# TinfoilHat0/Defending-Against-Backdoors-with-Robust-Learning-Rate

Hardware: NVIDIA H100
Metric: fl_rounds_per_sec (higher is better)
Workload: dtype bf16

## Files before the change

### defending-against-backdoors-with-robust-learning-rate_b200/ops/csrc/gemm.h

```cpp
#pragma once
#include <cuda_runtime.h>
#include <cuda_bf16.h>
#include <stdint.h>

#include "dropspec.h"

namespace rlr {

constexpr int kStatSlots = 16;

struct ConvGemmParams {
    int M, N, num_kb;
    int mode;
    int cblocks;
    int TW, TH, TN;
    int Ho, Wo, NB;
    int tiles_w, tiles_h;
    int ntaps;
    int in_stride;
    int out_stride, out_ph, out_pw, OutH, OutW;
    int8_t dh[9], dw[9];
    int dn[9];
    int b_mn;
    int wtap[9];
    int wcols;
    DropSpec drop;
    int tma_store;
    int split_prod;
    long long* dbg;
    const __nv_bfloat16* b_src;
    int b_ld, b_kvalid;
    const uint32_t* wait_flags;
    int wait_lo, wait_hi;
    const uint32_t* wait_epoch;
    void* out;
    int ldc;
    const float* bias;
    float* stats;
    int stat_slots;
    int relu, accumulate;
};

cudaError_t launch_gemm_bf16(const void* A, const void* B, void* out, int M, int N, int K, int lda, int ldb, int ldc,
                             const float* bias, int relu, int accumulate, float* stats, cudaStream_t st, const DropSpec* drop = nullptr);
cudaError_t launch_stem_gemm_bf16(const void* A, const void* W, void* out, int M, int N, int kvalid, int ldw, const float* bias, int relu,
                                  float* stats, const uint32_t* wait_flags, int wait_lo, int wait_hi, const uint32_t* wait_epoch,
                                  cudaStream_t st);
void set_pdl(int on);
cudaError_t launch_gemm_splitk_bf16(const void* A, const void* B, void* out, float* ws, int M, int N, int K, const float* bias, int relu,
                                    int num_sms, cudaStream_t st, const DropSpec* drop = nullptr);
void set_persistent_conv(int on);
void set_conv_occ3(int level);
void set_conv_tma_store(int on);
void set_conv_split_producer(int on);
void set_conv_trace(long long* buf);
long long* conv_trace_buf();
cudaError_t launch_conv_bf16(const void* x, const void* w, void* out, int NB, int planes, int Hin, int Win, int Cin, int Ho, int Wo,
                             int Cout, int ldc, int ntaps, const int* dh, const int* dw, const int* dplane, const float* bias,
                             int relu, int accumulate, float* stats, cudaStream_t st, const int* wtap = nullptr, int w_taps_total = 0,
                             int in_stride = 1, int out_stride = 1, int out_ph = 0, int out_pw = 0);

cudaError_t launch_conv3x3_halo_bf16(const void* x, const void* w, void* out, int NB, int Hin, int Win, int H, int W, int Cout, const float* bias,
                                     int relu, int accumulate, float* stats, int bo_mode, long long* dbg, int num_sms, cudaStream_t st);

cudaError_t launch_conv3x3_halo3_bf16(const void* x, const void* w, void* out, int NB, int H, int W, int Cout, const float* bias, int relu,
                                      int accumulate, int num_sms, cudaStream_t st);

cudaError_t launch_conv_wgrad_bf16(const void* dy, const void* x, float* dW, int NB, int planes, int Hin, int Win, int Cin, int Cin_valid,
                                   int Ho, int Wo, int Cout, int ntaps, const int* dh, const int* dw, const int* dplane, int num_sms,
                                   cudaStream_t st, int in_stride = 1);
cudaError_t launch_conv_wgrad_halo_bf16(const void* dy, const void* x, float* dW, int NB, int H, int W, int Cin_valid, int Cout,
                                        int num_sms, cudaStream_t st);
cudaError_t launch_linear_wgrad_bf16(const void* dy, const void* x, float* dW, int B, int N, int K, int num_sms, cudaStream_t st);

cudaError_t launch_ordered_sum_f32(float* out, const float* part, int nparts, long long n, cudaStream_t st);
cudaError_t launch_ordered_sum_f64(double* out, const double* part, int nparts, long long n, cudaStream_t st);
cudaError_t launch_channel_stats(const __nv_bfloat16* x, long long M, int C, float* stats , int num_sms, cudaStream_t st,
                                 int only_sum = 0, int nslots = 1);
cudaError_t launch_bn_finalize(const float* stats, int slots, float* mean_rstd, float* running_mean, float* running_var, int C,
                               float count, float eps, float momentum, int train, cudaStream_t st);
cudaError_t launch_bn_apply(const __nv_bfloat16* x, const __nv_bfloat16* res, __nv_bfloat16* y, const float* gamma, const float* beta,
                            float* mean_rstd, long long M, int C, int relu, int fin_mode, const float* stats, int slots, float count,
                            float eps, float momentum, float* running_mean, float* running_var, int num_sms, cudaStream_t st);
cudaError_t launch_bn_bwd_reduce(const __nv_bfloat16* dy, const __nv_bfloat16* y, const __nv_bfloat16* x, const float* mean_rstd,
                                 float* dsum , long long M, int C, int relu, int num_sms, cudaStream_t st,
                                 const float* gamma = nullptr, const float* beta = nullptr, int nslots = 1);
cudaError_t launch_bn_bwd_apply(const __nv_bfloat16* dy, const __nv_bfloat16* y, const __nv_bfloat16* x, const float* gamma,
                                const float* mean_rstd, const float* dsum, __nv_bfloat16* dx, __nv_bfloat16* dres, float* dgamma,
                                float* dbeta, long long M, int C, int relu, int num_sms, cudaStream_t st, const float* beta = nullptr, int nslots = 1);
cudaError_t launch_gn_fwd(const __nv_bfloat16* x, const __nv_bfloat16* res, __nv_bfloat16* y, const float* gamma, const float* beta,
                          float* mean_rstd, int B, int HW, int C, int G, float eps, int relu, int num_sms, cudaStream_t st);
cudaError_t launch_gn_bwd(const __nv_bfloat16* dy, const __nv_bfloat16* y, const __nv_bfloat16* x, const float* gamma,
                          const float* mean_rstd, __nv_bfloat16* dx, __nv_bfloat16* dres, float* dgamma, float* dbeta, int B, int HW,
                          int C, int G, int relu, int num_sms, cudaStream_t st);
cudaError_t launch_relu_bwd(__nv_bfloat16* dy, const __nv_bfloat16* y, long long n, int num_sms, cudaStream_t st, float scale = 1.0f);
cudaError_t launch_maxpool2_fwd(const __nv_bfloat16* x, __nv_bfloat16* y, uint8_t* idx, int B, int H, int W, int C, cudaStream_t st,
                                float drop_p = 0.f, uint64_t seed = 0, const long long* step = nullptr, uint64_t stream = 0);
cudaError_t launch_maxpool2_bwd(const __nv_bfloat16* dy, const uint8_t* idx, __nv_bfloat16* dx, int B, int H, int W, int C, cudaStream_t st,
                                float drop_p, uint64_t seed, const long long* step, uint64_t stream, const __nv_bfloat16* zmask);
cudaError_t launch_avgpool_fwd(const __nv_bfloat16* x, __nv_bfloat16* y, int B, int HW, int C, cudaStream_t st);
cudaError_t launch_avgpool_bwd(const __nv_bfloat16* dy, __nv_bfloat16* dx, int B, int HW, int C, cudaStream_t st);
cudaError_t launch_dropout_fwd(const __nv_bfloat16* x, __nv_bfloat16* y, uint8_t* mask, long long n, float p, uint64_t seed,
                               const long long* step, uint64_t stream, cudaStream_t st);
cudaError_t launch_dropout_bwd(const __nv_bfloat16* dy, const uint8_t* mask, __nv_bfloat16* dx, long long n, float p, cudaStream_t st);
cudaError_t launch_space_to_depth(const __nv_bfloat16* x, __nv_bfloat16* y, int NB, int H, int W, int C, int num_sms, cudaStream_t st);
cudaError_t launch_im2col_small(const __nv_bfloat16* x, __nv_bfloat16* A, int NB, int H, int W, int C, int Ho, int Wo, int k, int pad,
                                int num_sms, cudaStream_t st);
cudaError_t launch_depth_to_space(const __nv_bfloat16* x4, __nv_bfloat16* y, int NB, int H, int W, int C, int accumulate, int plane_mask,
                                  int num_sms, cudaStream_t st);
cudaError_t launch_filter_gather_transpose(const __nv_bfloat16* w, __nv_bfloat16* wt, int Cout, int T, int Cin, int nsub, const int* taps,
                                           cudaStream_t st);
cudaError_t launch_filter_transpose(const __nv_bfloat16* w, __nv_bfloat16* wt, int Cout, int ntaps, int Cin, cudaStream_t st);
cudaError_t launch_linear_small_fwd(const __nv_bfloat16* x, const __nv_bfloat16* w, const float* bias, __nv_bfloat16* y, int B, int K,
                                    int N, int relu, cudaStream_t st);
cudaError_t launch_linear_small_fwd2(const __nv_bfloat16* x, const __nv_bfloat16* w, const float* bias, __nv_bfloat16* y, int B, int K,
                                     int N, int relu, cudaStream_t st);
cudaError_t launch_linear_small_bwd2(const __nv_bfloat16* x, const __nv_bfloat16* dy, const __nv_bfloat16* w, __nv_bfloat16* dx,
                                     float* dw, float* db, int B, int K, int N, int accumulate_dx, cudaStream_t st);
cudaError_t launch_linear_small_bwd(const __nv_bfloat16* x, const __nv_bfloat16* dy, const __nv_bfloat16* w, __nv_bfloat16* dx,
                                    float* dw, float* db, int B, int K, int N, int accumulate_dx, cudaStream_t st);

}
```

### defending-against-backdoors-with-robust-learning-rate_b200/ops/csrc/gemm_binding.cpp

```cpp
#include <torch/extension.h>
#include <ATen/cuda/CUDAContext.h>
#include <c10/cuda/CUDAGuard.h>
#include <c10/cuda/CUDAStream.h>
#include <c10/cuda/CUDACachingAllocator.h>

#include <vector>

#include "gemm.h"

namespace rlr {
void* scratch_alloc(size_t bytes, cudaStream_t st) {
    return c10::cuda::CUDACachingAllocator::raw_alloc_with_stream(bytes < 256 ? 256 : bytes, st);
}
void scratch_free(void* p) { c10::cuda::CUDACachingAllocator::raw_delete(p); }
}

namespace {
inline cudaStream_t cur_stream() { return c10::cuda::getCurrentCUDAStream().stream(); }
inline int num_sms() { return at::cuda::getCurrentDeviceProperties()->multiProcessorCount; }
inline void check(cudaError_t e, const char* what) { TORCH_CHECK(e == cudaSuccess, what, ": ", cudaGetErrorString(e)); }
template <typename T>
inline T* opt(const c10::optional<at::Tensor>& t) { return t.has_value() && t->defined() ? reinterpret_cast<T*>(t->data_ptr()) : nullptr; }
inline const __nv_bfloat16* bf(const at::Tensor& t) {
    TORCH_CHECK(t.is_cuda() && t.scalar_type() == at::kBFloat16 && t.is_contiguous(), "expected contiguous CUDA bf16 tensor");
// ... 252 lines not shown
    check(rlr::launch_maxpool2_fwd(bf(x), bfm(y), (uint8_t*)idx.data_ptr(), x.size(0), x.size(1), x.size(2), x.size(3), cur_stream(),
                                   (float)drop_p, d.seed, d.step, d.stream), "maxpool2_fwd");
}
void maxpool2_bwd(at::Tensor dy, at::Tensor idx, at::Tensor dx, double drop_p, int64_t drop_seed, c10::optional<at::Tensor> drop_step, int64_t drop_stream,
                  c10::optional<at::Tensor> relu_out) {
    c10::cuda::CUDAGuard g(dx.device());
    const rlr::DropSpec d = drop_spec(drop_p, drop_seed, drop_step, drop_stream);
    const bool zm = relu_out.has_value() && relu_out->defined();
    TORCH_CHECK(!zm || (relu_out->scalar_type() == at::kBFloat16 && relu_out->is_contiguous() && relu_out->numel() == dy.numel()), "relu_out must match dy");
    TORCH_CHECK(dy.is_contiguous() && dx.is_contiguous() && idx.is_contiguous() && dy.size(1) == dx.size(1) / 2 && dy.size(2) == dx.size(2) / 2);
    check(rlr::launch_maxpool2_bwd(bf(dy), (const uint8_t*)idx.data_ptr(), bfm(dx), dx.size(0), dx.size(1), dx.size(2), dx.size(3), cur_stream(),
                                   (float)drop_p, d.seed, d.step, d.stream, zm ? bf(*relu_out) : nullptr), "maxpool2_bwd");
}
void avgpool_fwd(at::Tensor x, at::Tensor y) {
    c10::cuda::CUDAGuard g(x.device());
    check(rlr::launch_avgpool_fwd(bf(x), bfm(y), x.size(0), x.size(1) * x.size(2), x.size(3), cur_stream()), "avgpool_fwd");
}
void avgpool_bwd(at::Tensor dy, at::Tensor dx) {
    c10::cuda::CUDAGuard g(dx.device());
    check(rlr::launch_avgpool_bwd(bf(dy), bfm(dx), dx.size(0), dx.size(1) * dx.size(2), dx.size(3), cur_stream()), "avgpool_bwd");
}
void dropout_fwd(at::Tensor x, at::Tensor y, at::Tensor mask, double p, int64_t seed, at::Tensor step, int64_t stream) {
    c10::cuda::CUDAGuard g(x.device());
    check(rlr::launch_dropout_fwd(bf(x), bfm(y), (uint8_t*)mask.data_ptr(), x.numel(), (float)p, (uint64_t)seed,
                                  (const long long*)step.data_ptr(), (uint64_t)stream, cur_stream()), "dropout_fwd");
}
void dropout_bwd(at::Tensor dy, at::Tensor mask, at::Tensor dx, double p) {
    c10::cuda::CUDAGuard g(dx.device());
    check(rlr::launch_dropout_bwd(bf(dy), (const uint8_t*)mask.data_ptr(), bfm(dx), dx.numel(), (float)p, cur_stream()), "dropout_bwd");
}
void space_to_depth(at::Tensor x, at::Tensor y) {
    c10::cuda::CUDAGuard g(x.device());
    check(rlr::launch_space_to_depth(bf(x), bfm(y), x.size(0), x.size(1), x.size(2), x.size(3), num_sms(), cur_stream()), "space_to_depth");
}
void im2col_small(at::Tensor x, at::Tensor A, int64_t k, int64_t pad) {
    c10::cuda::CUDAGuard g(x.device());
    const int NB = x.size(0), H = x.size(1), W = x.size(2), C = x.size(3);
    const int Ho = H + 2 * pad - k + 1, Wo = W + 2 * pad - k + 1;
    TORCH_CHECK(x.dim() == 4 && x.is_contiguous() && A.is_contiguous() && A.numel() == (int64_t)NB * Ho * Wo * 64, "im2col_small: A must be [NB*Ho*Wo, 64]");
    check(rlr::launch_im2col_small(bf(x), bfm(A), NB, H, W, C, Ho, Wo, (int)k, (int)pad, num_sms(), cur_stream()), "im2col_small");
}
void depth_to_space(at::Tensor x4, at::Tensor y, bool accumulate, int64_t plane_mask) {
    c10::cuda::CUDAGuard g(y.device());
    check(rlr::launch_depth_to_space(bf(x4), bfm(y), y.size(0), y.size(1), y.size(2), y.size(3), accumulate, (int)plane_mask, num_sms(),
                                     cur_stream()), "depth_to_space");
}
void filter_gather_transpose(at::Tensor w, at::Tensor wt, int64_t Cout, int64_t T, int64_t Cin, std::vector<int64_t> taps) {
    c10::cuda::CUDAGuard g(w.device());
    int t[9];
    TORCH_CHECK(taps.size() >= 1 && taps.size() <= 9);
    for (size_t i = 0; i < taps.size(); ++i) t[i] = (int)taps[i];
    check(rlr::launch_filter_gather_transpose(bf(w), bfm(wt), Cout, T, Cin, (int)taps.size(), t, cur_stream()), "filter_gather_transpose");
}
void filter_transpose(at::Tensor w, at::Tensor wt, int64_t Cout, int64_t ntaps, int64_t Cin) {
    c10::cuda::CUDAGuard g(w.device());
    check(rlr::launch_filter_transpose(bf(w), bfm(wt), Cout, ntaps, Cin, cur_stream()), "filter_transpose");
}
void linear_small_fwd(at::Tensor x, at::Tensor w, c10::optional<at::Tensor> bias, at::Tensor y, bool relu) {
    c10::cuda::CUDAGuard g(x.device());
    check(rlr::launch_linear_small_fwd(bf(x), bf(w), opt<const float>(bias), bfm(y), x.size(0), x.size(1), w.size(0), relu, cur_stream()), "linear_small_fwd");
}
void linear_small_bwd(at::Tensor x, at::Tensor dy, at::Tensor w, c10::optional<at::Tensor> dx, at::Tensor dw, c10::optional<at::Tensor> db,
                      bool accumulate_dx) {
    c10::cuda::CUDAGuard g(x.device());
    check(rlr::launch_linear_small_bwd(bf(x), bf(dy), bf(w), const_cast<__nv_bfloat16*>(bfo(dx)), (float*)dw.data_ptr(), opt<float>(db),
                                       x.size(0), x.size(1), w.size(0), accumulate_dx, cur_stream()), "linear_small_bwd");
}
void linear_small_fwd2(at::Tensor x, at::Tensor w, c10::optional<at::Tensor> bias, at::Tensor y, bool relu) {
    c10::cuda::CUDAGuard g(x.device());
    check(rlr::launch_linear_small_fwd2(bf(x), bf(w), opt<const float>(bias), bfm(y), x.size(0), x.size(1), w.size(0), relu, cur_stream()), "linear_small_fwd2");
}
void linear_small_bwd2(at::Tensor x, at::Tensor dy, at::Tensor w, c10::optional<at::Tensor> dx, at::Tensor dw, c10::optional<at::Tensor> db,
                       bool accumulate_dx) {
    c10::cuda::CUDAGuard g(x.device());
    check(rlr::launch_linear_small_bwd2(bf(x), bf(dy), bf(w), const_cast<__nv_bfloat16*>(bfo(dx)), (float*)dw.data_ptr(), opt<float>(db),
                                        x.size(0), x.size(1), w.size(0), accumulate_dx, cur_stream()), "linear_small_bwd2");
}
}

void register_gemm_bindings(py::module_& m) {
    m.attr("STAT_SLOTS") = rlr::kStatSlots;
    m.def("set_persistent_conv", [](bool on) { rlr::set_persistent_conv(on ? 1 : 0); });
    m.def("set_pdl", [](bool on) { rlr::set_pdl(on ? 1 : 0); });
    m.def("set_conv_occ3", [](int64_t level) { rlr::set_conv_occ3((int)level); });
    m.def("set_conv_tma_store", [](bool on) { rlr::set_conv_tma_store(on ? 1 : 0); });
    m.def("set_conv_split_producer", [](bool on) { rlr::set_conv_split_producer(on ? 1 : 0); });
    m.def("set_conv_trace", [](c10::optional<at::Tensor> buf) {
        rlr::set_conv_trace(buf.has_value() && buf->defined() ? reinterpret_cast<long long*>(buf->data_ptr<int64_t>()) : nullptr);
    });
    m.def("gemm_bf16", &gemm_bf16, py::arg("A"), py::arg("B"), py::arg("out"), py::arg("bias"), py::arg("relu"), py::arg("accumulate"), py::arg("stats"),
          py::arg("drop_p") = 0.0, py::arg("drop_seed") = 0, py::arg("drop_step") = py::none(), py::arg("drop_stream") = 0);
    m.def("stem_gemm_bf16", &stem_gemm_bf16, py::arg("A"), py::arg("W"), py::arg("out"), py::arg("bias"), py::arg("relu"), py::arg("stats"),
          py::arg("ready_ptr") = 0, py::arg("lo") = 0, py::arg("hi") = 0, py::arg("epoch") = py::none());
    m.def("gemm_splitk_bf16", &gemm_splitk_bf16, py::arg("A"), py::arg("B"), py::arg("out"), py::arg("ws"), py::arg("bias"), py::arg("relu"),
          py::arg("drop_p") = 0.0, py::arg("drop_seed") = 0, py::arg("drop_step") = py::none(), py::arg("drop_stream") = 0);
    m.def("conv_bf16", &conv_bf16);
    m.def("conv_bf16_strided", &conv_bf16_strided);
    m.def("conv_wgrad_bf16_strided", &conv_wgrad_bf16_strided);
    m.def("conv3x3_halo_bf16", &conv3x3_halo_bf16);
    m.def("conv3x3_halo3_bf16", &conv3x3_halo3_bf16);
    m.def("conv_wgrad_bf16", &conv_wgrad_bf16);
    m.def("linear_wgrad_bf16", &linear_wgrad_bf16);
    m.def("conv_wgrad_halo_bf16", &conv_wgrad_halo_bf16);
    m.def("channel_stats", &channel_stats);
    m.def("ordered_sum", &ordered_sum);
    m.def("bias_grad", &bias_grad);
    m.def("bn_finalize", &bn_finalize);
    m.def("bn_apply", &bn_apply);
    m.def("bn_bwd", &bn_bwd);
    m.def("bn_bwd_recompute", &bn_bwd_recompute);
    m.def("gn_fwd", &gn_fwd);
    m.def("gn_bwd", &gn_bwd);
    m.def("relu_bwd", &relu_bwd, py::arg("dy"), py::arg("y"), py::arg("scale") = 1.0);
    m.def("maxpool2_fwd", &maxpool2_fwd, py::arg("x"), py::arg("y"), py::arg("idx"), py::arg("drop_p") = 0.0, py::arg("drop_seed") = 0,
          py::arg("drop_step") = py::none(), py::arg("drop_stream") = 0);
    m.def("maxpool2_bwd", &maxpool2_bwd, py::arg("dy"), py::arg("idx"), py::arg("dx"), py::arg("drop_p") = 0.0, py::arg("drop_seed") = 0,
          py::arg("drop_step") = py::none(), py::arg("drop_stream") = 0, py::arg("relu_out") = py::none());
    m.def("avgpool_fwd", &avgpool_fwd);
    m.def("avgpool_bwd", &avgpool_bwd);
    m.def("dropout_fwd", &dropout_fwd);
    m.def("dropout_bwd", &dropout_bwd);
    m.def("space_to_depth", &space_to_depth);
    m.def("im2col_small", &im2col_small);
    m.def("filter_transpose", &filter_transpose);
    m.def("depth_to_space", &depth_to_space);
    m.def("filter_gather_transpose", &filter_gather_transpose);
    m.def("linear_small_fwd", &linear_small_fwd);
    m.def("linear_small_bwd", &linear_small_bwd);
    m.def("linear_small_fwd2", &linear_small_fwd2);
    m.def("linear_small_bwd2", &linear_small_bwd2);
}
```

### defending-against-backdoors-with-robust-learning-rate_b200/ops/csrc/wgrad.cu

```cuda
#include <cuda.h>
#include <stdlib.h>

#include "common.cuh"
#include "gemm.h"
#include "wgmma.cuh"

namespace rlr {

using namespace wg;

cudaError_t make_tmap_bf16(CUtensorMap* map, const void* base, int rank, const uint64_t* dims, const uint64_t* strides_bytes,
                           const uint32_t* box, const uint32_t* elem_strides = nullptr);

constexpr int WG_BM = 128, WG_BK = 64;
constexpr int WG_STAGES = 3;
constexpr int WG_A_BYTES = 2 * 64 * WG_BK * 2;
constexpr int WG_THREADS = 256 + 32;
template <int BNW>
struct WgCfg {
    static constexpr int kGroups = BNW / 64;
    static constexpr int kBBytes = kGroups * 64 * WG_BK * 2;
    static constexpr int kStageBytes = WG_A_BYTES + 3 * kBBytes;
    static constexpr int kSmem = WG_STAGES * kStageBytes + 2048;
};

struct WgradParams {
    int mode;
    int num_kb;
    int kb_per_cta;
    int a_groups;
    int ntaps_cta;
    int T;
    int TW, TH, TN, tiles_w, tiles_h;
    int8_t dh[9], dw[9];
    int dn[9];
    int in_stride;
    int ci_tiles;
    int Cout, Cin_valid;
    float* dW;
    float* part;
};

struct __align__(8) WgShared {
    uint64_t full[WG_STAGES];
    uint64_t empty[WG_STAGES];
};

template <int NACC, int BNW>
__device__ __forceinline__ void wgrad_flush(const float (&acc)[NACC / 2], float* dW, float* part, int co, int Cout, int T, int tap0, int ci0,
                                            int Cin_valid, int t) {
    if (part) dW = part + (size_t)blockIdx.z * Cout * T * Cin_valid;
#pragma unroll
    for (int h = 0; h < 2; ++h) {
        const int row = co + 8 * h;
        if (row >= Cout) continue;
#pragma unroll
        for (int j = 0; j < NACC / 8; ++j) {
            const int c = frag_col(t, 4 * j), tap = c / BNW, ci = ci0 + c % BNW;
            float* dst = dW + ((size_t)row * T + tap0 + tap) * Cin_valid + ci;
            const float a = acc[4 * j + 2 * h], b = acc[4 * j + 2 * h + 1];
            if (part) {
                if (ci < Cin_valid) dst[0] = a;
                if (ci + 1 < Cin_valid) dst[1] = b;
            } else if ((Cin_valid & 1) == 0) {
                if (ci < Cin_valid) asm volatile("red.global.add.v2.f32 [%0], {%1, %2};" ::"l"(dst), "f"(a), "f"(b) : "memory");
            } else {
                if (ci < Cin_valid) atomicAdd(dst, a);
                if (ci + 1 < Cin_valid) atomicAdd(dst + 1, b);
            }
        }
    }
}

template <int BNW, int kTaps>
__global__ void __launch_bounds__(WG_THREADS, 1)
umma_wgrad_kernel(const __grid_constant__ CUtensorMap tmA, const __grid_constant__ CUtensorMap tmB, const WgradParams p) {
    using Cfg = WgCfg<BNW>;
    constexpr int WG_BN = BNW, WG_B_BYTES = Cfg::kBBytes, WG_STAGE_BYTES = Cfg::kStageBytes;
    constexpr int NACC = kTaps * BNW;
    extern __shared__ uint8_t smem_raw[];
    uint8_t* smem = reinterpret_cast<uint8_t*>((reinterpret_cast<uintptr_t>(smem_raw) + 1023) & ~uintptr_t(1023));
    WgShared* sh = reinterpret_cast<WgShared*>(smem + WG_STAGES * WG_STAGE_BYTES);
    const int warp = threadIdx.x >> 5, lane = threadIdx.x & 31;
    const int co_tile = blockIdx.x / p.ci_tiles, ci_tile = blockIdx.x - co_tile * p.ci_tiles;
    const int tap0 = blockIdx.y * kTaps;
    const int kb_begin = blockIdx.z * p.kb_per_cta;
    const int kb_end = min(p.num_kb, kb_begin + p.kb_per_cta);
    const int nkb = kb_end - kb_begin;

    if (warp == 8 && lane == 0) {
        prefetch_tmap(&tmA); prefetch_tmap(&tmB);
        for (int s = 0; s < WG_STAGES; ++s) { mbar_init(&sh->full[s], 1); mbar_init(&sh->empty[s], 8); }
        fence_barrier_init();
    }
    __syncthreads();
    pdl_wait();
    pdl_trigger();

    if (warp == 8) {
        if (lane == 0) {
            int stage = 0;
            uint32_t phase = 0;
            const uint32_t bytes = p.a_groups * 8192 + kTaps * WG_B_BYTES;
            for (int i = 0; i < nkb; ++i) {
                const int kb = kb_begin + i;
                mbar_wait(&sh->empty[stage], phase ^ 1);
                uint8_t* sa = smem + stage * WG_STAGE_BYTES;
                uint8_t* sb = sa + WG_A_BYTES;
                mbar_expect_tx(&sh->full[stage], bytes);
                if (p.mode == 1) {
                    const int tw_i = kb % p.tiles_w, th_i = (kb / p.tiles_w) % p.tiles_h, tn_i = kb / (p.tiles_w * p.tiles_h);
                    const int w0 = tw_i * p.TW, h0 = th_i * p.TH, n0 = tn_i * p.TN;
                    for (int g = 0; g < p.a_groups; ++g)
                        tma_load_4d(&tmA, &sh->full[stage], sa + g * 8192, co_tile * WG_BM + g * 64, w0, h0, n0);
                    for (int t = 0; t < kTaps; ++t)
                        for (int g = 0; g < Cfg::kGroups; ++g)
                            tma_load_4d(&tmB, &sh->full[stage], sb + t * WG_B_BYTES + g * 8192, ci_tile * WG_BN + g * 64,
                                        w0 * p.in_stride + p.dw[tap0 + t], h0 * p.in_stride + p.dh[tap0 + t], n0 + p.dn[tap0 + t]);
                } else {
                    for (int g = 0; g < p.a_groups; ++g)
                        tma_load_2d(&tmA, &sh->full[stage], sa + g * 8192, co_tile * WG_BM + g * 64, kb * WG_BK);
                    for (int g = 0; g < Cfg::kGroups; ++g)
                        tma_load_2d(&tmB, &sh->full[stage], sb + g * 8192, ci_tile * WG_BN + g * 64, kb * WG_BK);
                }
                if (++stage == WG_STAGES) { stage = 0; phase ^= 1; }
            }
        }
    } else if (nkb > 0) {
        const int wgi = threadIdx.x >> 7, t = threadIdx.x & 127;
        const bool active = wgi < p.a_groups;
        float acc[NACC / 2];
#pragma unroll
        for (int i = 0; i < NACC / 2; ++i) acc[i] = 0.f;
        int stage = 0, prev = -1;
        uint32_t phase = 0;
        for (int i = 0; i < nkb; ++i) {
            mbar_wait(&sh->full[stage], phase);
            if (active) {
                const uint32_t sa = smem_u32(smem + stage * WG_STAGE_BYTES) + wgi * 8192;
                const uint32_t sb = smem_u32(smem + stage * WG_STAGE_BYTES) + WG_A_BYTES;
                wgmma_fence();
#pragma unroll
                for (int k = 0; k < WG_BK / 16; ++k) {
                    wgmma_bf16<NACC, 1, 1>(acc, smem_desc_sw128(sa + k * 2048, 8192, 1024), smem_desc_sw128(sb + k * 2048, 8192, 1024),
                                           (i > 0 || k > 0) ? 1u : 0u);
                }
                wgmma_commit();
                wgmma_wait<1>();
            }
            if (prev >= 0 && lane == 0) mbar_arrive(&sh->empty[prev]);
            prev = stage;
            if (++stage == WG_STAGES) { stage = 0; phase ^= 1; }
        }
        if (active) {
            wgmma_wait<0>();
            fence_acc(acc);
            wgrad_flush<NACC, BNW>(acc, p.dW, p.part, co_tile * WG_BM + wgi * 64 + frag_row(t, 0), p.Cout, p.T, tap0, ci_tile * WG_BN, p.Cin_valid, t);
        }
    }
}

template <int BNW, int kTaps>
static cudaError_t launch_wg(const CUtensorMap& tmA, const CUtensorMap& tmB, WgradParams& p, int co_tiles, int tap_groups,
                             int num_sms, cudaStream_t st) {
    static bool configured = false;
    if (!configured) {
        RLR_CUDA_CHECK(cudaFuncSetAttribute(umma_wgrad_kernel<BNW, kTaps>, cudaFuncAttributeMaxDynamicSharedMemorySize, WgCfg<BNW>::kSmem));
        configured = true;
    }
    const int base = co_tiles * p.ci_tiles * tap_groups;
    static const int tune_waves = [] { const char* e = getenv("RLR_WG_WAVES"); return e ? atoi(e) : 0; }();
    int waves = base >= num_sms ? (base + num_sms - 1) / num_sms : (tune_waves > 0 ? tune_waves : 1);
    int splits = (waves * num_sms) / base;
    if (splits > p.num_kb) splits = p.num_kb;
    if (splits < 1) splits = 1;
    p.kb_per_cta = (p.num_kb + splits - 1) / splits;
    splits = (p.num_kb + p.kb_per_cta - 1) / p.kb_per_cta;
    dim3 grid(co_tiles * p.ci_tiles, tap_groups, splits);
    if (splits == 1) return launch_kernel(umma_wgrad_kernel<BNW, kTaps>, grid, dim3(WG_THREADS), (size_t)WgCfg<BNW>::kSmem, st, tmA, tmB, p);
    const long long plane = (long long)p.Cout * p.T * p.Cin_valid;
    Scratch part((size_t)splits * plane * sizeof(float), st);
    p.part = part.as<float>();
    RLR_CUDA_CHECK(launch_kernel(umma_wgrad_kernel<BNW, kTaps>, grid, dim3(WG_THREADS), (size_t)WgCfg<BNW>::kSmem, st, tmA, tmB, p));
    return launch_ordered_sum(p.dW, p.part, splits, plane, st);
}

constexpr int WH_STAGES = 3;
constexpr int WH_A_BYTES = 2 * 128 * 128;
constexpr int WH_HALO_BYTES = 18 * 16 * 128;
constexpr int WH_STAGE_BYTES = WH_A_BYTES + WH_HALO_BYTES;
constexpr int WH_SMEM = WH_STAGES * WH_STAGE_BYTES + 2048;

struct WgHaloParams {
    int NB, H, W, tiles_h, tiles_w;
    int num_kb, kb_per_cta;
    int a_groups;
    int Cout, Cin_valid;
    float* dW;
    float* part;
};

__global__ void __launch_bounds__(WG_THREADS, 1)
umma_wgrad_halo_kernel(const __grid_constant__ CUtensorMap tmA, const __grid_constant__ CUtensorMap tmB, const WgHaloParams p) {
    extern __shared__ uint8_t smem_raw[];
    uint8_t* smem = reinterpret_cast<uint8_t*>((reinterpret_cast<uintptr_t>(smem_raw) + 1023) & ~uintptr_t(1023));
    WgShared* sh = reinterpret_cast<WgShared*>(smem + WH_STAGES * WH_STAGE_BYTES);
    const int warp = threadIdx.x >> 5, lane = threadIdx.x & 31;
    const int co_tile = blockIdx.x;
    const int dy = blockIdx.y, tap0 = dy * 3;
    const int kb_begin = blockIdx.z * p.kb_per_cta;
    const int kb_end = min(p.num_kb, kb_begin + p.kb_per_cta);
    const int nkb = kb_end - kb_begin;
    const int tiles_per_img = p.tiles_h * p.tiles_w;

    if (warp == 8 && lane == 0) {
        prefetch_tmap(&tmA); prefetch_tmap(&tmB);
        for (int s = 0; s < WH_STAGES; ++s) { mbar_init(&sh->full[s], 1); mbar_init(&sh->empty[s], 8); }
        fence_barrier_init();
    }
    __syncthreads();
    pdl_wait();
    pdl_trigger();

    if (warp == 8) {
        if (lane == 0) {
            int stage = 0;
            uint32_t phase = 0;
            const uint32_t bytes = p.a_groups * 16384 + WH_HALO_BYTES;
            for (int i = 0; i < nkb; ++i) {
                const int kb = kb_begin + i;
                const int n = kb / tiles_per_img, r = kb - n * tiles_per_img;
                const int h0 = (r / p.tiles_w) * 16, w0 = (r % p.tiles_w) * 8;
                mbar_wait(&sh->empty[stage], phase ^ 1);
                uint8_t* sa = smem + stage * WH_STAGE_BYTES;
                mbar_expect_tx(&sh->full[stage], bytes);
                for (int g = 0; g < p.a_groups; ++g)
                    tma_load_4d(&tmA, &sh->full[stage], sa + g * 16384, co_tile * WG_BM + g * 64, w0, h0, n);
                tma_load_4d(&tmB, &sh->full[stage], sa + WH_A_BYTES, 0, w0 - 1, h0 - 1, n);
                if (++stage == WH_STAGES) { stage = 0; phase ^= 1; }
            }
        }
    } else if (nkb > 0) {
        const int wgi = threadIdx.x >> 7, t = threadIdx.x & 127;
        const bool active = wgi < p.a_groups;
        float acc[96];
#pragma unroll
        for (int i = 0; i < 96; ++i) acc[i] = 0.f;
        int stage = 0, prev = -1;
        uint32_t phase = 0;
        for (int i = 0; i < nkb; ++i) {
            mbar_wait(&sh->full[stage], phase);
            if (active) {
                const uint32_t sa = smem_u32(smem + stage * WH_STAGE_BYTES) + wgi * 16384;
                const uint32_t halo = smem_u32(smem + stage * WH_STAGE_BYTES) + WH_A_BYTES;
                wgmma_fence();
#pragma unroll
                for (int j = 0; j < 8; ++j) {
                    wgmma_bf16<192, 1, 1>(acc, smem_desc_sw128(sa + j * 2048, 16384, 1024),
                                          smem_desc_sw128(halo + ((2 * j + dy) * 16) * 128, 128, 2048), (i > 0 || j > 0) ? 1u : 0u);
                }
                wgmma_commit();
                wgmma_wait<1>();
            }
            if (prev >= 0 && lane == 0) mbar_arrive(&sh->empty[prev]);
            prev = stage;
            if (++stage == WH_STAGES) { stage = 0; phase ^= 1; }
        }
        if (active) {
            wgmma_wait<0>();
            fence_acc(acc);
            wgrad_flush<192, 64>(acc, p.dW, p.part, co_tile * WG_BM + wgi * 64 + frag_row(t, 0), p.Cout, 9, tap0, 0, p.Cin_valid, t);
        }
    }
}

cudaError_t launch_conv_wgrad_halo_bf16(const void* dy, const void* x, float* dW, int NB, int H, int W, int Cin_valid, int Cout,
                                        int num_sms, cudaStream_t st) {
    if (H % 16 || W % 8 || Cout % 8 || !((Cout <= 64) || Cout % 128 == 0)) return cudaErrorInvalidValue;
    static bool configured = false;
    if (!configured) {
        RLR_CUDA_CHECK(cudaFuncSetAttribute(umma_wgrad_halo_kernel, cudaFuncAttributeMaxDynamicSharedMemorySize, WH_SMEM));
        configured = true;
    }
    WgHaloParams p{};
    p.NB = NB; p.H = H; p.W = W; p.tiles_h = H / 16; p.tiles_w = W / 8; p.num_kb = NB * p.tiles_h * p.tiles_w;
    p.a_groups = (Cout % 128 == 0) ? 2 : 1; p.Cout = Cout; p.Cin_valid = Cin_valid; p.dW = dW;
    const int co_tiles = (Cout + WG_BM - 1) / WG_BM;
    const int base = co_tiles * 3;
    int waves = base >= num_sms ? (base + num_sms - 1) / num_sms : 1;
    int splits = (waves * num_sms) / base;
    if (splits > p.num_kb) splits = p.num_kb;
    if (splits < 1) splits = 1;
    p.kb_per_cta = (p.num_kb + splits - 1) / splits;
    splits = (p.num_kb + p.kb_per_cta - 1) / p.kb_per_cta;
    CUtensorMap tmA, tmB;
    {
        const uint64_t d[4] = {(uint64_t)Cout, (uint64_t)W, (uint64_t)H, (uint64_t)NB};
        const uint64_t s[3] = {(uint64_t)Cout * 2, (uint64_t)W * Cout * 2, (uint64_t)H * W * Cout * 2};
        const uint32_t b[4] = {64, 8, 16, 1};
        RLR_CUDA_CHECK(make_tmap_bf16(&tmA, dy, 4, d, s, b));
    }
    {
        const uint64_t d[4] = {64, (uint64_t)W, (uint64_t)H, (uint64_t)NB};
        const uint64_t s[3] = {128, (uint64_t)W * 128, (uint64_t)H * W * 128};
        const uint32_t b[4] = {64, 16, 18, 1};
        RLR_CUDA_CHECK(make_tmap_bf16(&tmB, x, 4, d, s, b));
    }
    if (splits == 1) return launch_kernel(umma_wgrad_halo_kernel, dim3(co_tiles, 3, splits), dim3(WG_THREADS), (size_t)WH_SMEM, st, tmA, tmB, p);
    const long long plane = (long long)Cout * 9 * Cin_valid;
    Scratch part((size_t)splits * plane * sizeof(float), st);
    p.part = part.as<float>();
    RLR_CUDA_CHECK(launch_kernel(umma_wgrad_halo_kernel, dim3(co_tiles, 3, splits), dim3(WG_THREADS), (size_t)WH_SMEM, st, tmA, tmB, p));
    return launch_ordered_sum(dW, p.part, splits, plane, st);
}

static int pow2_ceil_(int x) { int q = 1; while (q < x) q <<= 1; return q; }

cudaError_t launch_conv_wgrad_bf16(const void* dy, const void* x, float* dW, int NB, int planes, int Hin, int Win, int Cin, int Cin_valid,
                                   int Ho, int Wo, int Cout, int ntaps, const int* dh, const int* dw, const int* dplane, int num_sms,
                                   cudaStream_t st, int in_stride) {
    if (Cin % 64 || Cout % 8 || (ntaps != 1 && ntaps != 9)) return cudaErrorInvalidValue;
    if (in_stride < 1 || in_stride > 2 || (in_stride > 1 && planes != 1)) return cudaErrorInvalidValue;
    WgradParams p{};
    p.in_stride = in_stride;
    int TW = pow2_ceil_(Wo); if (TW > 64) TW = 64;
    int TH = pow2_ceil_(Ho); if (TW * TH > 64) TH = 64 / TW;
    const int TN = 64 / (TW * TH);
    p.mode = 1; p.TW = TW; p.TH = TH; p.TN = TN;
    p.tiles_w = (Wo + TW - 1) / TW; p.tiles_h = (Ho + TH - 1) / TH;
    p.num_kb = p.tiles_w * p.tiles_h * ((NB + TN - 1) / TN);
    p.T = ntaps; p.ntaps_cta = ntaps == 9 ? 3 : 1;
    for (int t = 0; t < ntaps; ++t) { p.dh[t] = (int8_t)dh[t]; p.dw[t] = (int8_t)dw[t]; p.dn[t] = dplane[t] * NB; }
    const bool wide = (Cin % 128 == 0) && (Cin_valid == Cin) && ntaps == 1;
    p.ci_tiles = wide ? Cin / 128 : Cin / 64; p.Cout = Cout; p.Cin_valid = Cin_valid; p.dW = dW;
    p.a_groups = Cout > 64 ? 2 : 1;
    const int co_tiles = (Cout + WG_BM - 1) / WG_BM;
    CUtensorMap tmA, tmB;
    {
        const uint64_t d[4] = {(uint64_t)Cout, (uint64_t)Wo, (uint64_t)Ho, (uint64_t)NB};
        const uint64_t s[3] = {(uint64_t)Cout * 2, (uint64_t)Wo * Cout * 2, (uint64_t)Ho * Wo * Cout * 2};
        const uint32_t b[4] = {64, (uint32_t)TW, (uint32_t)TH, (uint32_t)TN};
        RLR_CUDA_CHECK(make_tmap_bf16(&tmA, dy, 4, d, s, b));
    }
    {
        const uint64_t d[4] = {(uint64_t)Cin, (uint64_t)Win, (uint64_t)Hin, (uint64_t)planes * NB};
        const uint64_t s[3] = {(uint64_t)Cin * 2, (uint64_t)Win * Cin * 2, (uint64_t)Hin * Win * Cin * 2};
        const uint32_t b[4] = {64, (uint32_t)TW, (uint32_t)TH, (uint32_t)TN};
        const uint32_t es[4] = {1, (uint32_t)in_stride, (uint32_t)in_stride, 1};
        RLR_CUDA_CHECK(make_tmap_bf16(&tmB, x, 4, d, s, b, in_stride > 1 ? es : nullptr));
    }
    if (wide) return launch_wg<128, 1>(tmA, tmB, p, co_tiles, ntaps, num_sms, st);
    return ntaps == 9 ? launch_wg<64, 3>(tmA, tmB, p, co_tiles, 3, num_sms, st) : launch_wg<64, 1>(tmA, tmB, p, co_tiles, 1, num_sms, st);
}

cudaError_t launch_linear_wgrad_bf16(const void* dy, const void* x, float* dW, int B, int N, int K, int num_sms, cudaStream_t st) {
    if (N % 8 || K % 64) return cudaErrorInvalidValue;
    WgradParams p{};
    p.mode = 0; p.num_kb = (B + WG_BK - 1) / WG_BK; p.T = 1; p.ntaps_cta = 1; p.in_stride = 1;
    const bool wide = K % 128 == 0;
    p.ci_tiles = wide ? K / 128 : K / 64; p.Cout = N; p.Cin_valid = K; p.dW = dW;
    p.a_groups = N > 64 ? 2 : 1;
    const int co_tiles = (N + WG_BM - 1) / WG_BM;
    CUtensorMap tmA, tmB;
    {
        const uint64_t d[2] = {(uint64_t)N, (uint64_t)B}, s[1] = {(uint64_t)N * 2};
        const uint32_t b[2] = {64, WG_BK};
        RLR_CUDA_CHECK(make_tmap_bf16(&tmA, dy, 2, d, s, b));
    }
    {
        const uint64_t d[2] = {(uint64_t)K, (uint64_t)B}, s[1] = {(uint64_t)K * 2};
        const uint32_t b[2] = {64, WG_BK};
        RLR_CUDA_CHECK(make_tmap_bf16(&tmB, x, 2, d, s, b));
    }
    return wide ? launch_wg<128, 1>(tmA, tmB, p, co_tiles, 1, num_sms, st) : launch_wg<64, 1>(tmA, tmB, p, co_tiles, 1, num_sms, st);
}

}
```

Measured before the change: 0.6714.

## Load single halo tile per stage for 3x3 wgrad and deepen smem ring

Adds a halo mode to the generic conv wgrad kernel. For 3x3 tap blocks it issues one TMA load of a (TW+2)x(TH+2) input tile and addresses each tap through shifted wgmma descriptor offsets, instead of issuing three separate per-tap B loads. Stage counts are now derived from available shared memory, up to 8 stages, for both wgrad kernels, and the halo wgrad kernel is templated on its A-group count. This cuts redundant input traffic and TMA issue overhead and deepens pipelining, at the risk of descriptor layout errors for non-square tile widths.

```diff
diff --git a/defending-against-backdoors-with-robust-learning-rate_b200/ops/csrc/gemm.h b/defending-against-backdoors-with-robust-learning-rate_b200/ops/csrc/gemm.h
--- a/defending-against-backdoors-with-robust-learning-rate_b200/ops/csrc/gemm.h
+++ b/defending-against-backdoors-with-robust-learning-rate_b200/ops/csrc/gemm.h
@@ -71,6 +71,7 @@
                                    cudaStream_t st, int in_stride = 1);
 cudaError_t launch_conv_wgrad_halo_bf16(const void* dy, const void* x, float* dW, int NB, int H, int W, int Cin_valid, int Cout,
                                         int num_sms, cudaStream_t st);
+void set_wgrad_halo_any(int on);
 cudaError_t launch_linear_wgrad_bf16(const void* dy, const void* x, float* dW, int B, int N, int K, int num_sms, cudaStream_t st);
 
 cudaError_t launch_ordered_sum_f32(float* out, const float* part, int nparts, long long n, cudaStream_t st);
diff --git a/defending-against-backdoors-with-robust-learning-rate_b200/ops/csrc/gemm_binding.cpp b/defending-against-backdoors-with-robust-learning-rate_b200/ops/csrc/gemm_binding.cpp
--- a/defending-against-backdoors-with-robust-learning-rate_b200/ops/csrc/gemm_binding.cpp
+++ b/defending-against-backdoors-with-robust-learning-rate_b200/ops/csrc/gemm_binding.cpp
@@ -358,6 +358,7 @@
     m.attr("STAT_SLOTS") = rlr::kStatSlots;
     m.def("set_persistent_conv", [](bool on) { rlr::set_persistent_conv(on ? 1 : 0); });
     m.def("set_pdl", [](bool on) { rlr::set_pdl(on ? 1 : 0); });
+    m.def("set_wgrad_halo_any", [](bool on) { rlr::set_wgrad_halo_any(on ? 1 : 0); });
     m.def("set_conv_occ3", [](int64_t level) { rlr::set_conv_occ3((int)level); });
     m.def("set_conv_tma_store", [](bool on) { rlr::set_conv_tma_store(on ? 1 : 0); });
     m.def("set_conv_split_producer", [](bool on) { rlr::set_conv_split_producer(on ? 1 : 0); });
diff --git a/defending-against-backdoors-with-robust-learning-rate_b200/ops/csrc/wgrad.cu b/defending-against-backdoors-with-robust-learning-rate_b200/ops/csrc/wgrad.cu
--- a/defending-against-backdoors-with-robust-learning-rate_b200/ops/csrc/wgrad.cu
+++ b/defending-against-backdoors-with-robust-learning-rate_b200/ops/csrc/wgrad.cu
@@ -13,15 +13,19 @@
                            const uint32_t* box, const uint32_t* elem_strides = nullptr);
 
 constexpr int WG_BM = 128, WG_BK = 64;
-constexpr int WG_STAGES = 3;
 constexpr int WG_A_BYTES = 2 * 64 * WG_BK * 2;
 constexpr int WG_THREADS = 256 + 32;
-template <int BNW>
+constexpr int WG_HALO_MAX_BYTES = 34 * 4 * 128;
+constexpr int WG_MAX_STAGES = 8;
+constexpr int WG_SMEM_MAX = 227 * 1024;
+template <int BNW, int kTaps, bool kHalo = false>
 struct WgCfg {
     static constexpr int kGroups = BNW / 64;
     static constexpr int kBBytes = kGroups * 64 * WG_BK * 2;
-    static constexpr int kStageBytes = WG_A_BYTES + 3 * kBBytes;
-    static constexpr int kSmem = WG_STAGES * kStageBytes + 2048;
+    static constexpr int kStageBytes = WG_A_BYTES + (kHalo ? WG_HALO_MAX_BYTES : kTaps * kBBytes);
+    static constexpr int kStages = (WG_SMEM_MAX - 2048) / kStageBytes < WG_MAX_STAGES ? (WG_SMEM_MAX - 2048) / kStageBytes : WG_MAX_STAGES;
+    static constexpr int kSmem = kStages * kStageBytes + 2048;
+    static_assert(kStageBytes % 1024 == 0 && kStages >= 3 && kSmem <= WG_SMEM_MAX, "wgrad ring");
 };
 
 struct WgradParams {
@@ -35,6 +39,7 @@
     int8_t dh[9], dw[9];
     int dn[9];
     int in_stride;
+    int halo_bytes;
     int ci_tiles;
     int Cout, Cin_valid;
     float* dW;
@@ -42,8 +47,8 @@
 };
 
 struct __align__(8) WgShared {
-    uint64_t full[WG_STAGES];
-    uint64_t empty[WG_STAGES];
+    uint64_t full[WG_MAX_STAGES];
+    uint64_t empty[WG_MAX_STAGES];
 };
 
 template <int NACC, int BNW>
@@ -72,15 +77,16 @@
     }
 }
 
-template <int BNW, int kTaps>
+template <int BNW, int kTaps, bool kHalo>
 __global__ void __launch_bounds__(WG_THREADS, 1)
 umma_wgrad_kernel(const __grid_constant__ CUtensorMap tmA, const __grid_constant__ CUtensorMap tmB, const WgradParams p) {
-    using Cfg = WgCfg<BNW>;
-    constexpr int WG_BN = BNW, WG_B_BYTES = Cfg::kBBytes, WG_STAGE_BYTES = Cfg::kStageBytes;
+    static_assert(!kHalo || (BNW == 64 && kTaps == 3), "halo mode: one filter row of 64-channel taps");
+    using Cfg = WgCfg<BNW, kTaps, kHalo>;
+    constexpr int WG_BN = BNW, WG_B_BYTES = Cfg::kBBytes, WG_STAGE_BYTES = Cfg::kStageBytes, kStages = Cfg::kStages;
     constexpr int NACC = kTaps * BNW;
     extern __shared__ uint8_t smem_raw[];
     uint8_t* smem = reinterpret_cast<uint8_t*>((reinterpret_cast<uintptr_t>(smem_raw) + 1023) & ~uintptr_t(1023));
-    WgShared* sh = reinterpret_cast<WgShared*>(smem + WG_STAGES * WG_STAGE_BYTES);
+    WgShared* sh = reinterpret_cast<WgShared*>(smem + kStages * WG_STAGE_BYTES);
     const int warp = threadIdx.x >> 5, lane = threadIdx.x & 31;
     const int co_tile = blockIdx.x / p.ci_tiles, ci_tile = blockIdx.x - co_tile * p.ci_tiles;
     const int tap0 = blockIdx.y * kTaps;
@@ -90,7 +96,7 @@
 
     if (warp == 8 && lane == 0) {
         prefetch_tmap(&tmA); prefetch_tmap(&tmB);
-        for (int s = 0; s < WG_STAGES; ++s) { mbar_init(&sh->full[s], 1); mbar_init(&sh->empty[s], 8); }
+        for (int s = 0; s < kStages; ++s) { mbar_init(&sh->full[s], 1); mbar_init(&sh->empty[s], 8); }
         fence_barrier_init();
     }
     __syncthreads();
@@ -101,7 +107,7 @@
         if (lane == 0) {
             int stage = 0;
             uint32_t phase = 0;
-            const uint32_t bytes = p.a_groups * 8192 + kTaps * WG_B_BYTES;
+            const uint32_t bytes = p.a_groups * 8192 + (kHalo ? p.halo_bytes : kTaps * WG_B_BYTES);
             for (int i = 0; i < nkb; ++i) {
                 const int kb = kb_begin + i;
                 mbar_wait(&sh->empty[stage], phase ^ 1);
@@ -113,17 +119,21 @@
                     const int w0 = tw_i * p.TW, h0 = th_i * p.TH, n0 = tn_i * p.TN;
                     for (int g = 0; g < p.a_groups; ++g)
                         tma_load_4d(&tmA, &sh->full[stage], sa + g * 8192, co_tile * WG_BM + g * 64, w0, h0, n0);
-                    for (int t = 0; t < kTaps; ++t)
-                        for (int g = 0; g < Cfg::kGroups; ++g)
-                            tma_load_4d(&tmB, &sh->full[stage], sb + t * WG_B_BYTES + g * 8192, ci_tile * WG_BN + g * 64,
-                                        w0 * p.in_stride + p.dw[tap0 + t], h0 * p.in_stride + p.dh[tap0 + t], n0 + p.dn[tap0 + t]);
+                    if (kHalo) {
+                        tma_load_4d(&tmB, &sh->full[stage], sb, ci_tile * WG_BN, w0 + p.dw[0], h0 + p.dh[0], n0);
+                    } else {
+                        for (int t = 0; t < kTaps; ++t)
+                            for (int g = 0; g < Cfg::kGroups; ++g)
+                                tma_load_4d(&tmB, &sh->full[stage], sb + t * WG_B_BYTES + g * 8192, ci_tile * WG_BN + g * 64,
+                                            w0 * p.in_stride + p.dw[tap0 + t], h0 * p.in_stride + p.dh[tap0 + t], n0 + p.dn[tap0 + t]);
+                    }
                 } else {
                     for (int g = 0; g < p.a_groups; ++g)
                         tma_load_2d(&tmA, &sh->full[stage], sa + g * 8192, co_tile * WG_BM + g * 64, kb * WG_BK);
                     for (int g = 0; g < Cfg::kGroups; ++g)
                         tma_load_2d(&tmB, &sh->full[stage], sb + g * 8192, ci_tile * WG_BN + g * 64, kb * WG_BK);
                 }
-                if (++stage == WG_STAGES) { stage = 0; phase ^= 1; }
+                if (++stage == kStages) { stage = 0; phase ^= 1; }
             }
         }
     } else if (nkb > 0) {
@@ -132,6 +142,17 @@
         float acc[NACC / 2];
 #pragma unroll
         for (int i = 0; i < NACC / 2; ++i) acc[i] = 0.f;
+        uint32_t b_off[WG_BK / 16], b_lbo = 8192, b_sbo = 1024;
+#pragma unroll
+        for (int k = 0; k < WG_BK / 16; ++k) b_off[k] = k * 2048;
+        if (kHalo) {
+            const int pitch = p.TW + 2;
+#pragma unroll
+            for (int k = 0; k < WG_BK / 16; ++k)
+                b_off[k] = (((16 * k) / p.TW + (int)blockIdx.y) * pitch + (16 * k) % p.TW) * 128;
+            b_lbo = 128;
+            b_sbo = (p.TW == 8 ? pitch : 8) * 128;
+        }
         int stage = 0, prev = -1;
         uint32_t phase = 0;
         for (int i = 0; i < nkb; ++i) {
@@ -142,7 +163,7 @@
                 wgmma_fence();
 #pragma unroll
                 for (int k = 0; k < WG_BK / 16; ++k) {
-                    wgmma_bf16<NACC, 1, 1>(acc, smem_desc_sw128(sa + k * 2048, 8192, 1024), smem_desc_sw128(sb + k * 2048, 8192, 1024),
+                    wgmma_bf16<NACC, 1, 1>(acc, smem_desc_sw128(sa + k * 2048, 8192, 1024), smem_desc_sw128(sb + b_off[k], b_lbo, b_sbo),
                                            (i > 0 || k > 0) ? 1u : 0u);
                 }
                 wgmma_commit();
@@ -150,7 +171,7 @@
             }
             if (prev >= 0 && lane == 0) mbar_arrive(&sh->empty[prev]);
             prev = stage;
-            if (++stage == WG_STAGES) { stage = 0; phase ^= 1; }
+            if (++stage == kStages) { stage = 0; phase ^= 1; }
         }
         if (active) {
             wgmma_wait<0>();
@@ -160,12 +181,12 @@
     }
 }
 
-template <int BNW, int kTaps>
+template <int BNW, int kTaps, bool kHalo = false>
 static cudaError_t launch_wg(const CUtensorMap& tmA, const CUtensorMap& tmB, WgradParams& p, int co_tiles, int tap_groups,
                              int num_sms, cudaStream_t st) {
     static bool configured = false;
     if (!configured) {
-        RLR_CUDA_CHECK(cudaFuncSetAttribute(umma_wgrad_kernel<BNW, kTaps>, cudaFuncAttributeMaxDynamicSharedMemorySize, WgCfg<BNW>::kSmem));
+        RLR_CUDA_CHECK(cudaFuncSetAttribute(umma_wgrad_kernel<BNW, kTaps, kHalo>, cudaFuncAttributeMaxDynamicSharedMemorySize, WgCfg<BNW, kTaps, kHalo>::kSmem));
         configured = true;
     }
     const int base = co_tiles * p.ci_tiles * tap_groups;
@@ -177,31 +198,36 @@
     p.kb_per_cta = (p.num_kb + splits - 1) / splits;
     splits = (p.num_kb + p.kb_per_cta - 1) / p.kb_per_cta;
     dim3 grid(co_tiles * p.ci_tiles, tap_groups, splits);
-    if (splits == 1) return launch_kernel(umma_wgrad_kernel<BNW, kTaps>, grid, dim3(WG_THREADS), (size_t)WgCfg<BNW>::kSmem, st, tmA, tmB, p);
+    if (splits == 1) return launch_kernel(umma_wgrad_kernel<BNW, kTaps, kHalo>, grid, dim3(WG_THREADS), (size_t)WgCfg<BNW, kTaps, kHalo>::kSmem, st, tmA, tmB, p);
     const long long plane = (long long)p.Cout * p.T * p.Cin_valid;
     Scratch part((size_t)splits * plane * sizeof(float), st);
     p.part = part.as<float>();
-    RLR_CUDA_CHECK(launch_kernel(umma_wgrad_kernel<BNW, kTaps>, grid, dim3(WG_THREADS), (size_t)WgCfg<BNW>::kSmem, st, tmA, tmB, p));
+    RLR_CUDA_CHECK(launch_kernel(umma_wgrad_kernel<BNW, kTaps, kHalo>, grid, dim3(WG_THREADS), (size_t)WgCfg<BNW, kTaps, kHalo>::kSmem, st, tmA, tmB, p));
     return launch_ordered_sum(p.dW, p.part, splits, plane, st);
 }
 
-constexpr int WH_STAGES = 3;
-constexpr int WH_A_BYTES = 2 * 128 * 128;
 constexpr int WH_HALO_BYTES = 18 * 16 * 128;
-constexpr int WH_STAGE_BYTES = WH_A_BYTES + WH_HALO_BYTES;
-constexpr int WH_SMEM = WH_STAGES * WH_STAGE_BYTES + 2048;
+template <int kAGroups>
+struct WhCfg {
+    static constexpr int kABytes = kAGroups * 128 * 128;
+    static constexpr int kStageBytes = kABytes + WH_HALO_BYTES;
+    static constexpr int kStages = (WG_SMEM_MAX - 2048) / kStageBytes;
+    static constexpr int kSmem = kStages * kStageBytes + 2048;
+    static_assert(kStageBytes % 1024 == 0 && kStages >= 3 && kStages <= WG_MAX_STAGES, "wgrad halo ring");
+};
 
 struct WgHaloParams {
     int NB, H, W, tiles_h, tiles_w;
     int num_kb, kb_per_cta;
-    int a_groups;
     int Cout, Cin_valid;
     float* dW;
     float* part;
 };
 
+template <int kAGroups>
 __global__ void __launch_bounds__(WG_THREADS, 1)
 umma_wgrad_halo_kernel(const __grid_constant__ CUtensorMap tmA, const __grid_constant__ CUtensorMap tmB, const WgHaloParams p) {
+    constexpr int WH_STAGES = WhCfg<kAGroups>::kStages, WH_STAGE_BYTES = WhCfg<kAGroups>::kStageBytes, WH_A_BYTES = WhCfg<kAGroups>::kABytes;
     extern __shared__ uint8_t smem_raw[];
     uint8_t* smem = reinterpret_cast<uint8_t*>((reinterpret_cast<uintptr_t>(smem_raw) + 1023) & ~uintptr_t(1023));
     WgShared* sh = reinterpret_cast<WgShared*>(smem + WH_STAGES * WH_STAGE_BYTES);
@@ -226,7 +252,7 @@
         if (lane == 0) {
             int stage = 0;
             uint32_t phase = 0;
-            const uint32_t bytes = p.a_groups * 16384 + WH_HALO_BYTES;
+            const uint32_t bytes = kAGroups * 16384 + WH_HALO_BYTES;
             for (int i = 0; i < nkb; ++i) {
                 const int kb = kb_begin + i;
                 const int n = kb / tiles_per_img, r = kb - n * tiles_per_img;
@@ -234,7 +260,7 @@
                 mbar_wait(&sh->empty[stage], phase ^ 1);
                 uint8_t* sa = smem + stage * WH_STAGE_BYTES;
                 mbar_expect_tx(&sh->full[stage], bytes);
-                for (int g = 0; g < p.a_groups; ++g)
+                for (int g = 0; g < kAGroups; ++g)
                     tma_load_4d(&tmA, &sh->full[stage], sa + g * 16384, co_tile * WG_BM + g * 64, w0, h0, n);
                 tma_load_4d(&tmB, &sh->full[stage], sa + WH_A_BYTES, 0, w0 - 1, h0 - 1, n);
                 if (++stage == WH_STAGES) { stage = 0; phase ^= 1; }
@@ -242,7 +268,7 @@
         }
     } else if (nkb > 0) {
         const int wgi = threadIdx.x >> 7, t = threadIdx.x & 127;
-        const bool active = wgi < p.a_groups;
+        const bool active = wgi < kAGroups;
         float acc[96];
 #pragma unroll
         for (int i = 0; i < 96; ++i) acc[i] = 0.f;
@@ -279,12 +305,13 @@
     if (H % 16 || W % 8 || Cout % 8 || !((Cout <= 64) || Cout % 128 == 0)) return cudaErrorInvalidValue;
     static bool configured = false;
     if (!configured) {
-        RLR_CUDA_CHECK(cudaFuncSetAttribute(umma_wgrad_halo_kernel, cudaFuncAttributeMaxDynamicSharedMemorySize, WH_SMEM));
+        RLR_CUDA_CHECK(cudaFuncSetAttribute(umma_wgrad_halo_kernel<1>, cudaFuncAttributeMaxDynamicSharedMemorySize, WhCfg<1>::kSmem));
+        RLR_CUDA_CHECK(cudaFuncSetAttribute(umma_wgrad_halo_kernel<2>, cudaFuncAttributeMaxDynamicSharedMemorySize, WhCfg<2>::kSmem));
         configured = true;
     }
     WgHaloParams p{};
     p.NB = NB; p.H = H; p.W = W; p.tiles_h = H / 16; p.tiles_w = W / 8; p.num_kb = NB * p.tiles_h * p.tiles_w;
-    p.a_groups = (Cout % 128 == 0) ? 2 : 1; p.Cout = Cout; p.Cin_valid = Cin_valid; p.dW = dW;
+    p.Cout = Cout; p.Cin_valid = Cin_valid; p.dW = dW;
     const int co_tiles = (Cout + WG_BM - 1) / WG_BM;
     const int base = co_tiles * 3;
     int waves = base >= num_sms ? (base + num_sms - 1) / num_sms : 1;
@@ -306,15 +333,34 @@
         const uint32_t b[4] = {64, 16, 18, 1};
         RLR_CUDA_CHECK(make_tmap_bf16(&tmB, x, 4, d, s, b));
     }
-    if (splits == 1) return launch_kernel(umma_wgrad_halo_kernel, dim3(co_tiles, 3, splits), dim3(WG_THREADS), (size_t)WH_SMEM, st, tmA, tmB, p);
+    const bool two = Cout % 128 == 0;
+    auto launch = [&]() {
+        return two ? launch_kernel(umma_wgrad_halo_kernel<2>, dim3(co_tiles, 3, splits), dim3(WG_THREADS), (size_t)WhCfg<2>::kSmem, st, tmA, tmB, p)
+                   : launch_kernel(umma_wgrad_halo_kernel<1>, dim3(co_tiles, 3, splits), dim3(WG_THREADS), (size_t)WhCfg<1>::kSmem, st, tmA, tmB, p);
+    };
+    if (splits == 1) return launch();
     const long long plane = (long long)Cout * 9 * Cin_valid;
     Scratch part((size_t)splits * plane * sizeof(float), st);
     p.part = part.as<float>();
-    RLR_CUDA_CHECK(launch_kernel(umma_wgrad_halo_kernel, dim3(co_tiles, 3, splits), dim3(WG_THREADS), (size_t)WH_SMEM, st, tmA, tmB, p));
+    RLR_CUDA_CHECK(launch());
     return launch_ordered_sum(dW, p.part, splits, plane, st);
 }
 
 static int pow2_ceil_(int x) { int q = 1; while (q < x) q <<= 1; return q; }
+
+static int g_wgrad_halo_any = -1;
+void set_wgrad_halo_any(int on) { g_wgrad_halo_any = on ? 1 : 0; }
+static bool wgrad_halo_any() {
+    if (g_wgrad_halo_any < 0) { const char* e = getenv("RLR_WGRAD_HALO_ANY"); g_wgrad_halo_any = (e && atoi(e) == 0) ? 0 : 1; }
+    return g_wgrad_halo_any > 0;
+}
+
+static bool taps_are_3x3_block(int ntaps, const int* dh, const int* dw, const int* dplane) {
+    if (ntaps != 9) return false;
+    for (int t = 0; t < 9; ++t)
+        if (dh[t] != dh[0] + t / 3 || dw[t] != dw[0] + t % 3 || dplane[t] != 0) return false;
+    return true;
+}
 
 cudaError_t launch_conv_wgrad_bf16(const void* dy, const void* x, float* dW, int NB, int planes, int Hin, int Win, int Cin, int Cin_valid,
                                    int Ho, int Wo, int Cout, int ntaps, const int* dh, const int* dw, const int* dplane, int num_sms,
@@ -335,6 +381,9 @@
     p.ci_tiles = wide ? Cin / 128 : Cin / 64; p.Cout = Cout; p.Cin_valid = Cin_valid; p.dW = dW;
     p.a_groups = Cout > 64 ? 2 : 1;
     const int co_tiles = (Cout + WG_BM - 1) / WG_BM;
+    const bool halo = wgrad_halo_any() && taps_are_3x3_block(ntaps, dh, dw, dplane) && planes == 1 && in_stride == 1 && TN == 1 &&
+                      TW >= 8 && TW <= 32;
+    p.halo_bytes = halo ? (TW + 2) * (TH + 2) * 128 : 0;
     CUtensorMap tmA, tmB;
     {
         const uint64_t d[4] = {(uint64_t)Cout, (uint64_t)Wo, (uint64_t)Ho, (uint64_t)NB};
@@ -345,10 +394,11 @@
     {
         const uint64_t d[4] = {(uint64_t)Cin, (uint64_t)Win, (uint64_t)Hin, (uint64_t)planes * NB};
         const uint64_t s[3] = {(uint64_t)Cin * 2, (uint64_t)Win * Cin * 2, (uint64_t)Hin * Win * Cin * 2};
-        const uint32_t b[4] = {64, (uint32_t)TW, (uint32_t)TH, (uint32_t)TN};
+        const uint32_t b[4] = {64, (uint32_t)(halo ? TW + 2 : TW), (uint32_t)(halo ? TH + 2 : TH), (uint32_t)TN};
         const uint32_t es[4] = {1, (uint32_t)in_stride, (uint32_t)in_stride, 1};
         RLR_CUDA_CHECK(make_tmap_bf16(&tmB, x, 4, d, s, b, in_stride > 1 ? es : nullptr));
     }
+    if (halo) return launch_wg<64, 3, true>(tmA, tmB, p, co_tiles, 3, num_sms, st);
     if (wide) return launch_wg<128, 1>(tmA, tmB, p, co_tiles, ntaps, num_sms, st);
     return ntaps == 9 ? launch_wg<64, 3>(tmA, tmB, p, co_tiles, 3, num_sms, st) : launch_wg<64, 1>(tmA, tmB, p, co_tiles, 1, num_sms, st);
 }
```

After: 0.6884 (median of 6 runs). 1.03x the previous value.
